# automl/TransformersCanDoBayesianInference

Measured on NVIDIA H100. Metric: prior-sampled sequences/sec, full training step (prior sample + fwd + bwd + allreduce + clip + Adam), higher is better.
Workload: dtype bf16

## Files before the change

transformerscandobayesianinference_b200/csrc/attention_bwd_tc.cu:

```cuda
#include "attention_common.cuh"

namespace pfn {

constexpr int AB_ROWS = ATT_TILE_ROWS;
constexpr int AB_TILE = ATT_TILE;
constexpr int AB_THREADS = 3 * 128;
constexpr int AB_DQ_STAGES = 4;
constexpr int AB_DKV_STAGES = 3;
constexpr int AB_DQ_STAT_WARPS = 3;
constexpr int AB_DQ_OFF_RING = 4 * AB_TILE;
constexpr int AB_DQ_OFF_STAT = AB_DQ_OFF_RING + AB_DQ_STAGES * 2 * AB_TILE;
constexpr int AB_DQ_OFF_BAR = AB_DQ_OFF_STAT + 2 * 3 * 128 * 4;
constexpr int AB_DQ_SMEM = AB_DQ_OFF_BAR + (2 * AB_DQ_STAGES + 2 + 4) * 8 + 1024;
constexpr int AB_DKV_OFF_RING = 4 * AB_TILE;
constexpr int AB_DKV_OFF_STAT = AB_DKV_OFF_RING + AB_DKV_STAGES * 2 * AB_TILE;
constexpr int AB_DKV_OFF_BAR = AB_DKV_OFF_STAT + AB_DKV_STAGES * 2 * AB_ROWS * 4;
constexpr int AB_DKV_SMEM = AB_DKV_OFF_BAR + (2 * AB_DKV_STAGES + 1) * 8 + 1024;
static_assert(AB_DQ_SMEM <= 232448 && AB_DKV_SMEM <= 232448, "the tiles and rings must fit the 227 KB of shared memory");

struct AttnBwdParams {
  int T, B, H, sep;
  float scale, scale_log2;
  const __nv_bfloat16* qkv; int ld_qkv;
  const __nv_bfloat16* dout; int ld_dout;
  __nv_bfloat16* dqkv; int ld_dqkv;
  const float* lse;
  const float* delta;
  int delta_tm;
  float* dq_colsum;
  uint32_t drop_seed; int drop_thr;
  int n_tiles;
  int batch_major;
};

__device__ __forceinline__ float ab_delta(const AttnBwdParams& p, int b, int h, int i) {
  return p.delta_tm ? p.delta[att_tok(i, b, p.T, p.B, 0) * p.H + h] : p.delta[(static_cast<size_t>(b) * p.H + h) * p.T + i];
}

__global__ void __launch_bounds__(256)
attn_bwd_delta_kernel(const __nv_bfloat16* __restrict__ out, int ld_out, const __nv_bfloat16* __restrict__ dout,
                      int ld_dout, float* __restrict__ delta, int T, int B, int H, int batch_major) {
  const int lane = threadIdx.x & 31;
  const long long warp = (static_cast<long long>(blockIdx.x) * blockDim.x + threadIdx.x) >> 5;
  const long long nwarps = (static_cast<long long>(gridDim.x) * blockDim.x) >> 5;
  const long long rows = static_cast<long long>(T) * B;
  for (long long tok = warp; tok < rows; tok += nwarps) {
    const int t = batch_major ? static_cast<int>(tok % T) : static_cast<int>(tok / B);
    const int b = batch_major ? static_cast<int>(tok / T) : static_cast<int>(tok % B);
    for (int h0 = 0; h0 < H; h0 += 2) {
      const int h = h0 + (lane >> 4);
      float acc = 0.f;
      if (h < H) {
        const int col = h * ATT_DH + (lane & 15) * 8;
        const uint4 pa = *reinterpret_cast<const uint4*>(out + tok * ld_out + col);
        const uint4 pb = *reinterpret_cast<const uint4*>(dout + tok * ld_dout + col);
        const __nv_bfloat162* ha = reinterpret_cast<const __nv_bfloat162*>(&pa);
        const __nv_bfloat162* hb = reinterpret_cast<const __nv_bfloat162*>(&pb);
#pragma unroll
        for (int j = 0; j < 4; ++j) {
          const float2 x = __bfloat1622float2(ha[j]);
          const float2 y = __bfloat1622float2(hb[j]);
          acc = fmaf(x.x, y.x, acc);
          acc = fmaf(x.y, y.y, acc);
        }
      }
#pragma unroll
      for (int o = 8; o > 0; o >>= 1) acc += __shfl_xor_sync(0xffffffffu, acc, o);
      if ((lane & 15) == 0 && h < H) delta[(static_cast<size_t>(b) * H + h) * T + t] = acc;
    }
  }
}

__global__ void __launch_bounds__(AB_THREADS, 1)
attn_bwd_dq_kernel(const __grid_constant__ CUtensorMap tmQ, const __grid_constant__ CUtensorMap tmKV,
                   const __grid_constant__ CUtensorMap tmDO, const AttnBwdParams p) {
  extern __shared__ uint8_t smem_raw[];
  uint8_t* smem = att_smem_base(smem_raw);
  uint8_t* sQ = smem;
  uint8_t* sD = smem + 2 * AB_TILE;
  const AttPipe<AB_DQ_STAGES> pp(smem + AB_DQ_OFF_RING, reinterpret_cast<uint64_t*>(smem + AB_DQ_OFF_BAR));
  float* sStat = reinterpret_cast<float*>(smem + AB_DQ_OFF_STAT);
  uint64_t* st_full = pp.q_empty + 1;
  uint64_t* st_empty = st_full + 2;
  const int warp = threadIdx.x >> 5, lane = threadIdx.x & 31;
  const int E = p.H * ATT_DH;
  const int nblk = (p.sep + AB_ROWS - 1) / AB_ROWS;
  const int n_units = p.n_tiles * p.B * p.H;
  const float dscale = p.drop_thr > 0 ? drop_scale(p.drop_thr) : 1.0f;
  if (threadIdx.x == 0) {
    pp.init();
    for (int s = 0; s < 2; ++s) {
      tc::mbar_init(&st_full[s], 32 * AB_DQ_STAT_WARPS);
      tc::mbar_init(&st_empty[s], 256);
    }
    tc::mbar_fence_init();
  }
  __syncthreads();

  if (warp >= 8) {
    tc::setmaxnreg_dec<64>();
    if (warp > 8) {
      const int pw = warp - 9;
      for (int u = blockIdx.x, it = 0; u < n_units; u += gridDim.x, ++it) {
        const AttUnit unit = att_unit(u, p.n_tiles, p.H);
        const int sb = it & 1;
        float* st = sStat + sb * 3 * 128;
        tc::mbar_wait_suspend(&st_empty[sb], ((it >> 1) & 1) ^ 1);
#pragma unroll 1
        for (int r = pw + AB_DQ_STAT_WARPS * lane; r < 128; r += 32 * AB_DQ_STAT_WARPS) {
          const int i = unit.tile * 128 + r;
          const bool valid = i < p.T;
          st[r] = valid ? p.lse[static_cast<size_t>(unit.bh) * p.T + i] * 1.4426950408889634f : INFINITY;
          st[128 + r] = valid ? ab_delta(p, unit.b, unit.h, i) : 0.f;
        }
        __syncwarp();
        auto tok_of = [&](int r) { return att_tok(unit.tile * 128 + r, unit.b, p.T, p.B, p.batch_major); };
        auto load_row = [&](int r, uint4& xv, uint4& yv) {
          const int l = static_cast<int>(att_opaque(lane)), half = l >> 4, c8 = (l & 15) * 8;
          const size_t tok = tok_of(r);
          const __nv_bfloat16* qrow = p.qkv + tok * p.ld_qkv + unit.h * ATT_DH + c8;
          xv = *reinterpret_cast<const uint4*>(half ? p.dout + tok * p.ld_dout + unit.h * ATT_DH + c8 : qrow);
          yv = *reinterpret_cast<const uint4*>(qrow + (1 + half) * E);
        };
        auto finish_row = [&](int r, uint4 xv, uint4 yv) {
          const int l = static_cast<int>(att_opaque(lane)), half = l >> 4, c8 = (l & 15) * 8;
          const __nv_bfloat162* x2 = reinterpret_cast<const __nv_bfloat162*>(&xv);
          const __nv_bfloat162* y2 = reinterpret_cast<const __nv_bfloat162*>(&yv);
          float dot = 0.f;
#pragma unroll
          for (int c = 0; c < 4; ++c) {
            const float2 a = __bfloat1622float2(x2[c]), bb = __bfloat1622float2(y2[c]);
            dot = fmaf(a.x, bb.x, fmaf(a.y, bb.y, dot));
          }
#pragma unroll
          for (int o = 8; o > 0; o >>= 1) dot += __shfl_xor_sync(0xffffffffu, dot, o);
          const float sd = __shfl_sync(0xffffffffu, dot, 0), dpd = __shfl_sync(0xffffffffu, dot, 16);
          const int i = unit.tile * 128 + r;
          const float pr = fast_ex2(fmaf(sd, p.scale_log2, -st[r]));
          const float mk = p.drop_thr > 0 ? (drop_keep(p.drop_seed, static_cast<uint32_t>(unit.bh) * p.T + i, i, p.drop_thr) ? dscale : 0.f) : 1.f;
          const float ds = pr * fmaf(mk, dpd, -st[128 + r]) * p.scale;
          const float f = half ? pr * mk : ds;
          uint4 o;
          uint32_t* o32 = reinterpret_cast<uint32_t*>(&o);
#pragma unroll
          for (int c = 0; c < 4; ++c) {
            const float2 a = __bfloat1622float2(x2[c]);
            o32[c] = tc::pack_bf16x2(f * a.x, f * a.y);
          }
          *reinterpret_cast<uint4*>(p.dqkv + tok_of(r) * p.ld_dqkv + unit.h * ATT_DH + (1 + half) * E + c8) = o;
          if (lane == 0) st[256 + r] = ds;
        };
        const int r_lo = max(0, p.sep - unit.tile * 128), r_hi = min(128, p.T - unit.tile * 128);
        for (int r = r_lo + (pw - r_lo % AB_DQ_STAT_WARPS + AB_DQ_STAT_WARPS) % AB_DQ_STAT_WARPS; r < r_hi;
             r += 2 * AB_DQ_STAT_WARPS) {
          const int r2 = r + AB_DQ_STAT_WARPS < r_hi ? r + AB_DQ_STAT_WARPS : r;
          uint4 xa, ya, xb, yb;
          load_row(r, xa, ya);
          load_row(r2, xb, yb);
          finish_row(r, xa, ya);
          if (r2 != r) finish_row(r2, xb, yb);
        }
        tc::mbar_arrive(&st_full[sb]);
      }
    } else if (threadIdx.x == 256) {
      tc::tma_prefetch_desc(&tmQ);
      tc::tma_prefetch_desc(&tmKV);
      tc::tma_prefetch_desc(&tmDO);
      att_kv_producer(pp, &tmKV, n_units, p.n_tiles, p.H, nblk, 4 * AB_TILE, [&](const AttUnit& unit) {
        for (int g = 0; g < 2; ++g) {
          const int t0 = unit.tile * 128 + 64 * g;
          att_load_tile(sQ + g * AB_TILE, &tmQ, pp.q_full, unit.h * ATT_DH, unit.b, t0);
          att_load_tile(sD + g * AB_TILE, &tmDO, pp.q_full, unit.h * ATT_DH, unit.b, t0);
        }
      });
    }
    return;
  }

  tc::setmaxnreg_inc<208>();
  const int g = warp >> 2, wq = warp & 3;
  const uint32_t q_tile = tc::smem_u32(sQ + g * AB_TILE), d_tile = tc::smem_u32(sD + g * AB_TILE);
  AttRing<AB_DQ_STAGES> ring;
  bool timed_out = false;
  for (int u = blockIdx.x, it = 0; u < n_units && !timed_out; u += gridDim.x, ++it) {
    const AttUnit unit = att_unit(u, p.n_tiles, p.H);
    const int i0 = unit.tile * 128 + 64 * g + 16 * wq + (lane >> 2);

    const int sb = it & 1;
    if (!tc::mbar_wait_bounded(&st_full[sb], (it >> 1) & 1)) { timed_out = true; break; }
    float lse2[2], dl[2], dsd[2];
    uint32_t drow[2];
#pragma unroll
    for (int r = 0; r < 2; ++r) {
      const int rr = i0 + 8 * r - unit.tile * 128;
      lse2[r] = sStat[sb * 3 * 128 + rr];
      dl[r] = sStat[sb * 3 * 128 + 128 + rr];
      dsd[r] = sStat[sb * 3 * 128 + 256 + rr];
      drow[r] = static_cast<uint32_t>(unit.bh) * p.T + i0 + 8 * r;
    }
    tc::mbar_arrive(&st_empty[sb]);

    float dq[64], s[32], dp[32];
    uint32_t ads[16];
    auto issue_sdp = [&](int st) {
      const uint32_t k_s = tc::smem_u32(pp.ring + st * 2 * AB_TILE);
      const uint32_t v_s = k_s + AB_TILE;
      const uint32_t q_s = att_opaque(q_tile), d_s = att_opaque(d_tile);
      tc::wgmma_fence();
#pragma unroll
      for (int kk = 0; kk < 8; ++kk) att_mma_n64(s, att_desc_k(q_s, kk), att_desc_k(k_s, kk), kk);
#pragma unroll
      for (int kk = 0; kk < 8; ++kk) att_mma_n64(dp, att_desc_k(d_s, kk), att_desc_k(v_s, kk), kk);
      tc::wgmma_commit();
    };
    auto issue_dq = [&](int st, bool accumulate) {
      const uint32_t k_s = tc::smem_u32(pp.ring + st * 2 * AB_TILE);
      tc::wgmma_fence();
#pragma unroll
      for (int kk = 0; kk < 4; ++kk) tc::wgmma_m64n128k16_rs(dq, ads + 4 * kk, att_desc_mn(k_s, kk), accumulate || kk > 0);
      tc::wgmma_commit();
    };
    auto compute_ds = [&](int kb) {
      const int key0 = kb * AB_ROWS + 2 * (lane & 3);
#pragma unroll
      for (int e = 0; e < 32; ++e) {
        const int r = (e >> 1) & 1;
        const int key = key0 + 8 * (e >> 2) + (e & 1);
        const float pr = key < p.sep ? fast_ex2(fmaf(s[e], p.scale_log2, -lse2[r])) : 0.f;
        const float mk = p.drop_thr > 0 ? (drop_keep(p.drop_seed, drow[r], key, p.drop_thr) ? dscale : 0.f) : 1.f;
        s[e] = pr * fmaf(mk, dp[e], -dl[r]) * p.scale;
      }
    };
    auto pack_ds = [&]() {
#pragma unroll
      for (int e = 0; e < 16; ++e) ads[e] = tc::pack_bf16x2(s[2 * e], s[2 * e + 1]);
    };
    uint32_t kd[2][16];
    auto load_kd = [&]() {
#pragma unroll
      for (int r = 0; r < 2; ++r) {
        const int i = i0 + 8 * r;
        const bool diag = i < p.T && i >= p.sep;
        const __nv_bfloat16* krow = p.qkv + att_tok(diag ? i : 0, unit.b, p.T, p.B, p.batch_major) * p.ld_qkv + E + unit.h * ATT_DH;
#pragma unroll
        for (int j = 0; j < 16; ++j)
          kd[r][j] = diag ? *reinterpret_cast<const uint32_t*>(krow + 8 * j + 2 * (lane & 3)) : 0u;
      }
    };
    if (att_key_loop(pp, ring, it, nblk, issue_sdp, issue_dq, [&] { tc::wgmma_fence_regs(s); tc::wgmma_fence_regs(dp); },
                     [&] { tc::wgmma_fence_regs(dq); }, compute_ds, pack_ds, load_kd)) {
      timed_out = true;
      break;
    }

    float cs[16][2];
#pragma unroll
    for (int j = 0; j < 16; ++j) cs[j][0] = cs[j][1] = 0.f;
#pragma unroll
    for (int r = 0; r < 2; ++r) {
      const int i = i0 + 8 * r;
      if (i < p.T) {
        const bool diag = i >= p.sep;
        __nv_bfloat16* grow = p.dqkv + att_tok(i, unit.b, p.T, p.B, p.batch_major) * p.ld_dqkv + unit.h * ATT_DH;
#pragma unroll
        for (int j = 0; j < 16; ++j) {
          float x = nblk > 0 ? dq[4 * j + 2 * r] : 0.f, y = nblk > 0 ? dq[4 * j + 2 * r + 1] : 0.f;
          if (diag) {
            const float2 k = __bfloat1622float2(*reinterpret_cast<const __nv_bfloat162*>(&kd[r][j]));
            x = fmaf(dsd[r], k.x, x);
            y = fmaf(dsd[r], k.y, y);
          }
          att_st2(grow, j, lane, x, y);
          cs[j][0] += __bfloat162float(__float2bfloat16_rn(x));
          cs[j][1] += __bfloat162float(__float2bfloat16_rn(y));
        }
      }
    }
    if (p.dq_colsum != nullptr) {
#pragma unroll
      for (int j = 0; j < 16; ++j)
#pragma unroll
        for (int e = 0; e < 2; ++e) {
          float v = cs[j][e];
          v += __shfl_xor_sync(0xffffffffu, v, 4);
          v += __shfl_xor_sync(0xffffffffu, v, 8);
          v += __shfl_xor_sync(0xffffffffu, v, 16);
          if (lane < 4) atomicAdd(p.dq_colsum + unit.h * ATT_DH + 8 * j + 2 * lane + e, v);
        }
    }
  }
  if (timed_out) asm volatile("trap;");
}

__global__ void __launch_bounds__(AB_THREADS, 1)
attn_bwd_dkv_kernel(const __grid_constant__ CUtensorMap tmQ, const __grid_constant__ CUtensorMap tmKV,
                    const __grid_constant__ CUtensorMap tmDO, const AttnBwdParams p) {
  extern __shared__ uint8_t smem_raw[];
  uint8_t* smem = att_smem_base(smem_raw);
  uint8_t* sK = smem;
  uint8_t* sV = smem + 2 * AB_TILE;
  uint8_t* sRing = smem + AB_DKV_OFF_RING;
  float* sStat = reinterpret_cast<float*>(smem + AB_DKV_OFF_STAT);
  uint64_t* full = reinterpret_cast<uint64_t*>(smem + AB_DKV_OFF_BAR);
  uint64_t* empty = full + AB_DKV_STAGES;
  uint64_t* kv_bar = empty + AB_DKV_STAGES;
  const int warp = threadIdx.x >> 5, lane = threadIdx.x & 31;
  const AttUnit unit = att_unit(blockIdx.x, p.n_tiles, p.H);
  const int E = p.H * ATT_DH;
  const int nqb = (p.T + AB_ROWS - 1) / AB_ROWS;
  if (threadIdx.x == 0) {
    for (int s = 0; s < AB_DKV_STAGES; ++s) {
      tc::mbar_init(&full[s], 1 + AB_ROWS);
      tc::mbar_init(&empty[s], 2);
    }
    tc::mbar_init(kv_bar, 1);
    tc::mbar_fence_init();
  }
  __syncthreads();

  if (warp >= 8) {
    tc::setmaxnreg_dec<40>();
    const int pt = threadIdx.x - 256;
    AttRing<AB_DKV_STAGES> ring;
    if (pt == 0) {
      tc::tma_prefetch_desc(&tmQ);
      tc::tma_prefetch_desc(&tmKV);
      tc::tma_prefetch_desc(&tmDO);
      tc::mbar_expect_tx(kv_bar, 4 * AB_TILE);
      for (int g = 0; g < 2; ++g) {
        const int j0 = unit.tile * 128 + 64 * g;
        att_load_tile(sK + g * AB_TILE, &tmKV, kv_bar, E + unit.h * ATT_DH, unit.b, j0);
        att_load_tile(sV + g * AB_TILE, &tmKV, kv_bar, 2 * E + unit.h * ATT_DH, unit.b, j0);
// ... 149 lines not shown
```

transformerscandobayesianinference_b200/csrc/attention_common.cuh:

```cuda
#pragma once
#include "common.cuh"
#include "dropout.cuh"
#include "tc_common.cuh"
#include "../../include/pfn_b200.h"

namespace pfn {

constexpr int ATT_DH = 128;
constexpr int ATT_ROW_BYTES = ATT_DH * 2;
constexpr int ATT_TILE_ROWS = 64;
constexpr int ATT_TILE = ATT_TILE_ROWS * ATT_ROW_BYTES;

int check_attn_desc_public(const pfn_attn_desc* d, bool bwd, const char* who);

__device__ __forceinline__ size_t att_tok(int t, int b, int T, int B, int batch_major) {
  return batch_major ? static_cast<size_t>(b) * T + t : static_cast<size_t>(t) * B + b;
}

__device__ __forceinline__ uint64_t att_desc_k(uint32_t tile, int kk) {
  return tc::wgmma_smem_desc(tile + (kk >> 2) * 8192 + (kk & 3) * 32, 16, 1024);
}
__device__ __forceinline__ uint64_t att_desc_mn(uint32_t tile, int kk) {
  return tc::wgmma_smem_desc(tile + kk * 2048, 8192, 1024);
}
__device__ __forceinline__ uint32_t att_opaque(uint32_t addr) {
  asm volatile("" : "+r"(addr));
  return addr;
}
__device__ __forceinline__ void att_mma_n64(float (&d)[32], uint64_t a_desc, uint64_t b_desc, int kk) {
  if (kk == 0) tc::wgmma_m64n64k16<0>(d, a_desc, b_desc);
  else tc::wgmma_m64n64k16<1>(d, a_desc, b_desc);
}

__device__ __forceinline__ void att_load_tile(uint8_t* dst, const CUtensorMap* m, uint64_t* bar, int col0, int b, int t0) {
  tc::tma_load_3d(dst, m, bar, col0, b, t0);
  tc::tma_load_3d(dst + 8192, m, bar, col0 + 64, b, t0);
}

struct AttUnit {
  int tile;
  int bh, h, b;
};
__device__ __forceinline__ AttUnit att_unit(int u, int n_tiles, int H) {
  const int bh = u / n_tiles;
  return {u % n_tiles, bh, bh % H, bh / H};
}

template <int STAGES>
struct AttRing {
  int stage = 0;
  uint32_t phase = 0;
  __device__ __forceinline__ void advance() { if (++stage == STAGES) { stage = 0; phase ^= 1; } }
};

__device__ __forceinline__ uint8_t* att_smem_base(uint8_t* raw) {
  return raw + ((1024u - (tc::smem_u32(raw) & 1023u)) & 1023u);
}

template <int STAGES>
struct AttPipe {
  uint8_t* ring;
  uint64_t* kv_full;
  uint64_t* kv_empty;
  uint64_t* q_full;
  uint64_t* q_empty;
  __device__ __forceinline__ AttPipe(uint8_t* ring_smem, uint64_t* bars)
      : ring(ring_smem), kv_full(bars), kv_empty(bars + STAGES), q_full(bars + 2 * STAGES), q_empty(bars + 2 * STAGES + 1) {}
  __device__ __forceinline__ void init() const {
    for (int s = 0; s < STAGES; ++s) {
      tc::mbar_init(&kv_full[s], 1);
      tc::mbar_init(&kv_empty[s], 2);
    }
    tc::mbar_init(q_full, 1);
    tc::mbar_init(q_empty, 2);
  }
};

template <int STAGES, class LoadQ>
__device__ __forceinline__ void att_kv_producer(const AttPipe<STAGES>& pp, const CUtensorMap* tmKV, int n_units, int n_tiles,
                                                int H, int nblk, uint32_t q_bytes, LoadQ&& load_q) {
  const int E = H * ATT_DH;
  AttRing<STAGES> ring;
  for (int u = blockIdx.x, it = 0; u < n_units; u += gridDim.x, ++it) {
    const AttUnit unit = att_unit(u, n_tiles, H);
    auto claim_q = [&]() {
      if (it > 0) tc::mbar_wait_suspend(pp.q_empty, (it - 1) & 1);
      tc::mbar_expect_tx(pp.q_full, q_bytes);
      load_q(unit);
    };
    const int claim_at = min(STAGES - 1, nblk - 1);
    if (nblk == 0) claim_q();
    for (int kb = 0; kb < nblk; ++kb) {
      if (kb == claim_at) claim_q();
      tc::mbar_wait_suspend(&pp.kv_empty[ring.stage], ring.phase ^ 1);
      uint8_t* dst = pp.ring + ring.stage * 2 * ATT_TILE;
      tc::mbar_expect_tx(&pp.kv_full[ring.stage], 2 * ATT_TILE);
      att_load_tile(dst, tmKV, &pp.kv_full[ring.stage], E + unit.h * ATT_DH, unit.b, kb * ATT_TILE_ROWS);
      att_load_tile(dst + ATT_TILE, tmKV, &pp.kv_full[ring.stage], 2 * E + unit.h * ATT_DH, unit.b, kb * ATT_TILE_ROWS);
      ring.advance();
    }
  }
}

template <int STAGES, class IssueA, class IssueB, class FenceA, class FenceB, class Math, class Pack, class BeforeTail>
__device__ __forceinline__ bool att_key_loop(const AttPipe<STAGES>& pp, AttRing<STAGES>& ring, int it, int nblk,
                                             IssueA&& issue_a, IssueB&& issue_b, FenceA&& fence_a, FenceB&& fence_b,
                                             Math&& math, Pack&& pack, BeforeTail&& before_tail) {
  const bool leader = (threadIdx.x & 127) == 0;
  if (!tc::mbar_wait_bounded(pp.q_full, it & 1)) return true;
  if (nblk > 0) {
    if (!tc::mbar_wait_bounded(&pp.kv_full[ring.stage], ring.phase)) return true;
    issue_a(ring.stage);
    tc::wgmma_wait<0>();
    fence_a();
    if (nblk == 1 && leader) tc::mbar_arrive(pp.q_empty);
    math(0);
    pack();
    int cur = ring.stage;
    ring.advance();
    bool timed_out = false;
    for (int kb = 1; kb < nblk; ++kb) {
      if (!timed_out && !tc::mbar_wait_bounded(&pp.kv_full[ring.stage], ring.phase)) timed_out = true;
      issue_a(ring.stage);
      issue_b(cur, kb > 1);
      tc::wgmma_wait<1>();
      fence_a();
      if (kb == nblk - 1 && leader) tc::mbar_arrive(pp.q_empty);
      math(kb);
      tc::wgmma_wait<0>();
      fence_b();
      if (leader) tc::mbar_arrive(&pp.kv_empty[cur]);
      cur = ring.stage;
      ring.advance();
      pack();
    }
    issue_b(cur, nblk > 1);
    before_tail();
    tc::wgmma_wait<0>();
    fence_b();
    if (timed_out) return true;
    if (leader) tc::mbar_arrive(&pp.kv_empty[cur]);
  } else {
    if (leader) tc::mbar_arrive(pp.q_empty);
    before_tail();
  }
  return false;
}

__device__ __forceinline__ float2 att_ld2(const __nv_bfloat16* row, int j, int lane) {
  return __bfloat1622float2(*reinterpret_cast<const __nv_bfloat162*>(row + 8 * j + 2 * (lane & 3)));
}
__device__ __forceinline__ void att_st2(__nv_bfloat16* row, int j, int lane, float x, float y) {
  *reinterpret_cast<uint32_t*>(row + 8 * j + 2 * (lane & 3)) = tc::pack_bf16x2(x, y);
}
__device__ __forceinline__ float quad_sum(float v) {
  v += __shfl_xor_sync(0xffffffffu, v, 1);
  return v + __shfl_xor_sync(0xffffffffu, v, 2);
}
__device__ __forceinline__ float quad_max(float v) {
  v = fmaxf(v, __shfl_xor_sync(0xffffffffu, v, 1));
  return fmaxf(v, __shfl_xor_sync(0xffffffffu, v, 2));
}

static inline int check_tc_attn(const pfn_attn_desc* d, bool bwd, const char* who) {
  if (int rc = check_attn_desc_public(d, bwd, who)) return rc;
  PFN_CHECK_ARG(d->dtype == PFN_BF16, "%s: bf16 only", who);
  PFN_CHECK_ARG(d->dh == ATT_DH, "%s: head dim %d unsupported (built for 128)", who, d->dh);
  PFN_CHECK_ARG(d->ld_qkv % 8 == 0 && d->ld_out % 8 == 0, "%s: leading dims must be multiples of 8", who);
  PFN_CHECK_ARG(((reinterpret_cast<uintptr_t>(d->qkv) | reinterpret_cast<uintptr_t>(d->out)) & 15) == 0,
                "%s: qkv/out must be 16-byte aligned", who);
  if (bwd) {
    PFN_CHECK_ARG(d->ld_dout % 8 == 0 && d->ld_dqkv % 8 == 0, "%s: leading dims must be multiples of 8", who);
    PFN_CHECK_ARG(((reinterpret_cast<uintptr_t>(d->dout) | reinterpret_cast<uintptr_t>(d->dqkv)) & 15) == 0,
                  "%s: dout/dqkv must be 16-byte aligned", who);
  }
  return 0;
}

template <auto Kernel, class... Args>
static inline int att_launch_persistent(const char* who, long long units, int threads, int smem, cudaStream_t s,
                                        const Args&... args) {
  PFN_CHECK_ARG(units < (1LL << 31), "%s: too many tiles", who);
  static bool attr_set[64] = {};
  if (first_use_on_device(attr_set)) PFN_CUDA_OK(cudaFuncSetAttribute(Kernel, cudaFuncAttributeMaxDynamicSharedMemorySize, smem));
  const int grid = units < num_sms() ? static_cast<int>(units) : num_sms();
  Kernel<<<static_cast<unsigned>(grid), threads, smem, s>>>(args...);
  PFN_LAUNCH_OK();
  return 0;
}

static inline int att_tensor_map(CUtensorMap* m, const void* base, int cols, int ld, int T, int B, int t_extent,
                                 int batch_major) {
  const uint64_t row = static_cast<uint64_t>(ld) * 2;
  const uint64_t dims[3] = {static_cast<uint64_t>(cols), static_cast<uint64_t>(B), static_cast<uint64_t>(t_extent)};
  const uint64_t strides[3] = {0, batch_major ? row * T : row, batch_major ? row : row * B};
  const uint32_t box[3] = {64, 1, ATT_TILE_ROWS};
  return make_tensor_map(m, base, false, 3, dims, strides, box, true);
}

static inline int att_qkv_maps(const pfn_attn_desc* d, CUtensorMap* tmQ, CUtensorMap* tmKV) {
  const int E = d->H * ATT_DH;
  if (int rc = att_tensor_map(tmQ, d->qkv, 3 * E, d->ld_qkv, d->T, d->B, d->T, d->batch_major)) return rc;
  return att_tensor_map(tmKV, d->qkv, 3 * E, d->ld_qkv, d->T, d->B, d->sep > 0 ? d->sep : 1, d->batch_major);
}

}
```

transformerscandobayesianinference_b200/csrc/attention_tc.cu:

```cuda
#include "attention_common.cuh"

namespace pfn {

constexpr int AF_THREADS = 3 * 128;
constexpr int AF_STAGES = 4;
constexpr int AF_OFF_STG = 2 * ATT_TILE;
constexpr int AF_OFF_RING = 4 * ATT_TILE;
constexpr int AF_OFF_BAR = AF_OFF_RING + AF_STAGES * 2 * ATT_TILE;
constexpr int AF_SMEM = AF_OFF_BAR + (2 * AF_STAGES + 2) * 8 + 1024;
static_assert(AF_SMEM <= 232448, "the tiles and the ring must fit the 227 KB of shared memory");

struct AttnFwdParams {
  int T, B, H, sep;
  float scale_log2;
  const __nv_bfloat16* qkv; int ld_qkv;
  float* lse;
  int n_tiles;
  int batch_major;
  uint32_t drop_seed; int drop_thr;
};

__global__ void __launch_bounds__(AF_THREADS, 1)
attn_fwd_kernel(const __grid_constant__ CUtensorMap tmQ, const __grid_constant__ CUtensorMap tmKV,
                const __grid_constant__ CUtensorMap tmO, const AttnFwdParams p) {
  extern __shared__ uint8_t smem_raw[];
  uint8_t* smem = att_smem_base(smem_raw);
  uint8_t* sQ = smem;
  uint8_t* sStg = smem + AF_OFF_STG;
  const AttPipe<AF_STAGES> pp(smem + AF_OFF_RING, reinterpret_cast<uint64_t*>(smem + AF_OFF_BAR));
  const int warp = threadIdx.x >> 5, lane = threadIdx.x & 31;
  const int E = p.H * ATT_DH;
  const int nblk = (p.sep + ATT_TILE_ROWS - 1) / ATT_TILE_ROWS;
  const int n_units = p.n_tiles * p.B * p.H;
  if (threadIdx.x == 0) {
    pp.init();
    tc::mbar_fence_init();
  }
  __syncthreads();

  if (warp >= 8) {
    tc::setmaxnreg_dec<40>();
    if (threadIdx.x == 256) {
      tc::tma_prefetch_desc(&tmQ);
      tc::tma_prefetch_desc(&tmKV);
      att_kv_producer(pp, &tmKV, n_units, p.n_tiles, p.H, nblk, 2 * ATT_TILE, [&](const AttUnit& unit) {
        for (int g = 0; g < 2; ++g)
          att_load_tile(sQ + g * ATT_TILE, &tmQ, pp.q_full, unit.h * ATT_DH, unit.b, unit.tile * 128 + 64 * g);
      });
    }
    return;
  }

  tc::setmaxnreg_inc<232>();
  const int g = warp >> 2, wq = warp & 3;
  const int tid = threadIdx.x & 127;
  const uint32_t q_tile = tc::smem_u32(sQ + g * ATT_TILE);
  uint8_t* stg = sStg + g * ATT_TILE;
  const float dscale = p.drop_thr > 0 ? drop_scale(p.drop_thr) : 1.0f;
  AttRing<AF_STAGES> ring;
  bool timed_out = false;
  for (int u = blockIdx.x, it = 0; u < n_units && !timed_out; u += gridDim.x, ++it) {
    const AttUnit unit = att_unit(u, p.n_tiles, p.H);
    const int t0 = unit.tile * 128 + 64 * g;
    const int i0 = t0 + 16 * wq + (lane >> 2);

    float o[64], m[2], l[2];
    uint32_t drow[2];
#pragma unroll
    for (int r = 0; r < 2; ++r) {
      const int i = i0 + 8 * r;
      const bool diag = i < p.T && i >= p.sep;
      drow[r] = static_cast<uint32_t>(unit.bh) * p.T + i;
      const __nv_bfloat16* qrow = p.qkv + att_tok(diag ? i : 0, unit.b, p.T, p.B, p.batch_major) * p.ld_qkv + unit.h * ATT_DH;
      float sd = 0.f;
      if (diag) {
#pragma unroll
        for (int j = 0; j < 16; ++j) {
          const float2 q = att_ld2(qrow, j, lane), k = att_ld2(qrow + E, j, lane);
          sd = fmaf(q.x, k.x, fmaf(q.y, k.y, sd));
        }
      }
      sd = quad_sum(sd) * p.scale_log2;
      m[r] = diag ? sd : -INFINITY;
      l[r] = diag && (lane & 3) == 0 ? 1.f : 0.f;
      const bool keep = diag && (p.drop_thr == 0 || drop_keep(p.drop_seed, drow[r], i, p.drop_thr));
#pragma unroll
      for (int j = 0; j < 16; ++j) {
        const float2 v = keep ? att_ld2(qrow + 2 * E, j, lane) : make_float2(0.f, 0.f);
        o[4 * j + 2 * r] = v.x;
        o[4 * j + 2 * r + 1] = v.y;
      }
    }

    float s[32];
    uint32_t ap[16];
    float corr[2];
    auto issue_s = [&](int st) {
      const uint32_t k_s = tc::smem_u32(pp.ring + st * 2 * ATT_TILE);
      const uint32_t q_s = att_opaque(q_tile);
      tc::wgmma_fence();
#pragma unroll
      for (int kk = 0; kk < 8; ++kk) att_mma_n64(s, att_desc_k(q_s, kk), att_desc_k(k_s, kk), kk);
      tc::wgmma_commit();
    };
    auto issue_pv = [&](int st, bool) {
      const uint32_t v_s = tc::smem_u32(pp.ring + st * 2 * ATT_TILE) + ATT_TILE;
      tc::wgmma_fence();
#pragma unroll
      for (int kk = 0; kk < 4; ++kk) tc::wgmma_m64n128k16_rs(o, ap + 4 * kk, att_desc_mn(v_s, kk), 1);
      tc::wgmma_commit();
    };
    auto softmax = [&](int kb) {
      const int key0 = kb * ATT_TILE_ROWS + 2 * (lane & 3);
      if (kb * ATT_TILE_ROWS + ATT_TILE_ROWS > p.sep) {
#pragma unroll
        for (int e = 0; e < 32; ++e)
          if (key0 + 8 * (e >> 2) + (e & 1) >= p.sep) s[e] = -INFINITY;
      }
      float mx[2] = {-INFINITY, -INFINITY};
#pragma unroll
      for (int e = 0; e < 32; ++e) mx[(e >> 1) & 1] = fmaxf(mx[(e >> 1) & 1], s[e]);
#pragma unroll
      for (int r = 0; r < 2; ++r) {
        const float mn = fmaxf(m[r], quad_max(mx[r]) * p.scale_log2);
        corr[r] = fast_ex2(m[r] - mn);
        m[r] = mn;
        l[r] *= corr[r];
      }
#pragma unroll
      for (int e = 0; e < 32; ++e) {
        const int r = (e >> 1) & 1;
        const float pr = fast_ex2(fmaf(s[e], p.scale_log2, -m[r]));
        l[r] += pr;
        s[e] = p.drop_thr > 0 && !drop_keep(p.drop_seed, drow[r], key0 + 8 * (e >> 2) + (e & 1), p.drop_thr) ? 0.f : pr;
      }
    };
    auto rescale_pack = [&]() {
#pragma unroll
      for (int e = 0; e < 64; ++e) o[e] *= corr[(e >> 1) & 1];
#pragma unroll
      for (int e = 0; e < 16; ++e) ap[e] = tc::pack_bf16x2(s[2 * e], s[2 * e + 1]);
    };
    if (att_key_loop(pp, ring, it, nblk, issue_s, issue_pv, [&] { tc::wgmma_fence_regs(s); },
                     [&] { tc::wgmma_fence_regs(o); }, softmax, rescale_pack, [] {})) {
      timed_out = true;
      break;
    }

    if (tid == 0) tc::bulk_wait_read<0>();
    tc::named_bar_sync(1 + g, 128);
#pragma unroll
    for (int r = 0; r < 2; ++r) {
      const int i = i0 + 8 * r;
      const float lr = quad_sum(l[r]);
      const float inv = dscale / lr;
      const int rr = 16 * wq + (lane >> 2) + 8 * r;
#pragma unroll
      for (int j = 0; j < 16; ++j) {
        const uint32_t off = (j >> 3) * 8192 + rr * 128 + (((j & 7) ^ (rr & 7)) << 4) + (lane & 3) * 4;
        *reinterpret_cast<uint32_t*>(stg + off) = tc::pack_bf16x2(o[4 * j + 2 * r] * inv, o[4 * j + 2 * r + 1] * inv);
      }
      if (i < p.T && (lane & 3) == 0) p.lse[static_cast<size_t>(unit.bh) * p.T + i] = (m[r] + __log2f(lr)) * 0.69314718055994531f;
    }
    tc::fence_proxy_async_smem();
    tc::named_bar_sync(1 + g, 128);
    if (tid == 0 && t0 < p.T) {
      tc::tma_store_3d(&tmO, stg, unit.h * ATT_DH, unit.b, t0);
      tc::tma_store_3d(&tmO, stg + 8192, unit.h * ATT_DH + 64, unit.b, t0);
      tc::bulk_commit();
    }
  }
  if (tid == 0) tc::bulk_wait<0>();
  if (timed_out) asm volatile("trap;");
}

}

using namespace pfn;

extern "C" int pfn_attention_fwd_tc(const pfn_attn_desc* d, void* stream) {
  if (int rc = check_tc_attn(d, false, "attention_fwd_tc")) return rc;
  AttnFwdParams p;
  p.T = d->T; p.B = d->B; p.H = d->H; p.sep = d->sep;
  p.scale_log2 = d->scale * 1.4426950408889634f;
  p.qkv = reinterpret_cast<const __nv_bfloat16*>(d->qkv); p.ld_qkv = d->ld_qkv;
  p.lse = d->lse;
  p.n_tiles = (d->T + 127) / 128;
  p.batch_major = d->batch_major;
  p.drop_seed = d->drop_seed; p.drop_thr = d->drop_thr;
  const int E = d->H * ATT_DH;
  CUtensorMap tmQ, tmKV, tmO;
  if (int rc = att_qkv_maps(d, &tmQ, &tmKV)) return rc;
  if (int rc = att_tensor_map(&tmO, d->out, E, d->ld_out, d->T, d->B, d->T, d->batch_major)) return rc;
  return att_launch_persistent<attn_fwd_kernel>("attention_fwd_tc", static_cast<long long>(p.n_tiles) * d->B * d->H,
                                                AF_THREADS, AF_SMEM, reinterpret_cast<cudaStream_t>(stream), tmQ, tmKV, tmO, p);
}
```

transformerscandobayesianinference_b200/csrc/tc_common.cuh:

```cuda
#pragma once
#include <cuda.h>
#include <cuda_bf16.h>
#include <cuda_runtime.h>
#include <stdint.h>

namespace pfn {
namespace tc {

__device__ __forceinline__ uint32_t smem_u32(const void* p) {
  return static_cast<uint32_t>(__cvta_generic_to_shared(p));
}

__device__ __forceinline__ void mbar_init(uint64_t* bar, uint32_t count) {
  asm volatile("mbarrier.init.shared::cta.b64 [%0], %1;" ::"r"(smem_u32(bar)), "r"(count) : "memory");
}
__device__ __forceinline__ void mbar_fence_init() {
  asm volatile("fence.mbarrier_init.release.cluster;" ::: "memory");
}
__device__ __forceinline__ void mbar_expect_tx(uint64_t* bar, uint32_t bytes) {
  asm volatile("mbarrier.arrive.expect_tx.shared::cta.b64 _, [%0], %1;" ::"r"(smem_u32(bar)), "r"(bytes) : "memory");
}
__device__ __forceinline__ void mbar_arrive(uint64_t* bar) {
  asm volatile("mbarrier.arrive.shared::cta.b64 _, [%0];" ::"r"(smem_u32(bar)) : "memory");
}
// ... 71 lines not shown
}
__device__ __forceinline__ void bulk_commit() { asm volatile("cp.async.bulk.commit_group;" ::: "memory"); }
template <int N>
__device__ __forceinline__ void bulk_wait_read() {
  asm volatile("cp.async.bulk.wait_group.read %0;" ::"n"(N) : "memory");
}
template <int N>
__device__ __forceinline__ void bulk_wait() {
  asm volatile("cp.async.bulk.wait_group %0;" ::"n"(N) : "memory");
}
__device__ __forceinline__ void fence_proxy_async_smem() { asm volatile("fence.proxy.async.shared::cta;" ::: "memory"); }

__device__ __forceinline__ void named_bar_sync(int id, int threads) {
  asm volatile("bar.sync %0, %1;" ::"r"(id), "r"(threads) : "memory");
}
__device__ __forceinline__ void named_bar_arrive(int id, int threads) {
  asm volatile("bar.arrive %0, %1;" ::"r"(id), "r"(threads) : "memory");
}
template <int N>
__device__ __forceinline__ void setmaxnreg_dec() { asm volatile("setmaxnreg.dec.sync.aligned.u32 %0;" ::"n"(N)); }
template <int N>
__device__ __forceinline__ void setmaxnreg_inc() { asm volatile("setmaxnreg.inc.sync.aligned.u32 %0;" ::"n"(N)); }

__device__ __forceinline__ uint32_t pack_bf16x2(float lo, float hi) {
  __nv_bfloat162 t = __floats2bfloat162_rn(lo, hi);
  return *reinterpret_cast<uint32_t*>(&t);
}

__device__ __forceinline__ uint64_t wgmma_smem_desc(uint32_t smem_addr, uint32_t lbo_bytes, uint32_t sbo_bytes) {
  return (1ull << 62) | (static_cast<uint64_t>((sbo_bytes >> 4) & 0x3FFF) << 32) |
         (static_cast<uint64_t>((lbo_bytes >> 4) & 0x3FFF) << 16) | static_cast<uint64_t>((smem_addr >> 4) & 0x3FFF);
}

__device__ __forceinline__ void wgmma_fence() { asm volatile("wgmma.fence.sync.aligned;" ::: "memory"); }
__device__ __forceinline__ void wgmma_commit() { asm volatile("wgmma.commit_group.sync.aligned;" ::: "memory"); }
template <int N>
__device__ __forceinline__ void wgmma_wait() {
  asm volatile("wgmma.wait_group.sync.aligned %0;" ::"n"(N) : "memory");
}
template <int N>
__device__ __forceinline__ void wgmma_fence_regs(float (&d)[N]) {
#pragma unroll
  for (int i = 0; i < N; ++i) asm volatile("" : "+f"(d[i])::"memory");
}

template <int TA, int TB>
__device__ __forceinline__ void wgmma_m64n128k16(float (&d)[64], uint64_t a_desc, uint64_t b_desc, uint32_t accumulate) {
  asm volatile(
      "{\n\t.reg .pred p;\n\t"
      "setp.ne.b32 p, %66, 0;\n\t"
      "wgmma.mma_async.sync.aligned.m64n128k16.f32.bf16.bf16 "
      "{%0, %1, %2, %3, %4, %5, %6, %7, %8, %9, %10, %11, %12, %13, %14, %15, "
      "%16, %17, %18, %19, %20, %21, %22, %23, %24, %25, %26, %27, %28, %29, %30, %31, "
      "%32, %33, %34, %35, %36, %37, %38, %39, %40, %41, %42, %43, %44, %45, %46, %47, "
      "%48, %49, %50, %51, %52, %53, %54, %55, %56, %57, %58, %59, %60, %61, %62, %63}, "
      "%64, %65, p, 1, 1, %67, %68;\n\t}"
      : "+f"(d[0]), "+f"(d[1]), "+f"(d[2]), "+f"(d[3]), "+f"(d[4]), "+f"(d[5]), "+f"(d[6]), "+f"(d[7]),
        "+f"(d[8]), "+f"(d[9]), "+f"(d[10]), "+f"(d[11]), "+f"(d[12]), "+f"(d[13]), "+f"(d[14]), "+f"(d[15]),
        "+f"(d[16]), "+f"(d[17]), "+f"(d[18]), "+f"(d[19]), "+f"(d[20]), "+f"(d[21]), "+f"(d[22]), "+f"(d[23]),
        "+f"(d[24]), "+f"(d[25]), "+f"(d[26]), "+f"(d[27]), "+f"(d[28]), "+f"(d[29]), "+f"(d[30]), "+f"(d[31]),
        "+f"(d[32]), "+f"(d[33]), "+f"(d[34]), "+f"(d[35]), "+f"(d[36]), "+f"(d[37]), "+f"(d[38]), "+f"(d[39]),
        "+f"(d[40]), "+f"(d[41]), "+f"(d[42]), "+f"(d[43]), "+f"(d[44]), "+f"(d[45]), "+f"(d[46]), "+f"(d[47]),
        "+f"(d[48]), "+f"(d[49]), "+f"(d[50]), "+f"(d[51]), "+f"(d[52]), "+f"(d[53]), "+f"(d[54]), "+f"(d[55]),
        "+f"(d[56]), "+f"(d[57]), "+f"(d[58]), "+f"(d[59]), "+f"(d[60]), "+f"(d[61]), "+f"(d[62]), "+f"(d[63])
      : "l"(a_desc), "l"(b_desc), "r"(accumulate), "n"(TA), "n"(TB));
}

#define PFN_WGMMA_D32(C)                                                                                          \
  C(d[0]), C(d[1]), C(d[2]), C(d[3]), C(d[4]), C(d[5]), C(d[6]), C(d[7]), C(d[8]), C(d[9]), C(d[10]), C(d[11]),   \
      C(d[12]), C(d[13]), C(d[14]), C(d[15]), C(d[16]), C(d[17]), C(d[18]), C(d[19]), C(d[20]), C(d[21]),         \
      C(d[22]), C(d[23]), C(d[24]), C(d[25]), C(d[26]), C(d[27]), C(d[28]), C(d[29]), C(d[30]), C(d[31])
#define PFN_WGMMA_M64N64K16(SCALE_D)                                                                              \
  "wgmma.mma_async.sync.aligned.m64n64k16.f32.bf16.bf16 "                                                         \
  "{%0, %1, %2, %3, %4, %5, %6, %7, %8, %9, %10, %11, %12, %13, %14, %15, "                                       \
  "%16, %17, %18, %19, %20, %21, %22, %23, %24, %25, %26, %27, %28, %29, %30, %31}, %32, %33, " SCALE_D ", 1, 1, 0, 0;"
template <int ACCUMULATE>
__device__ __forceinline__ void wgmma_m64n64k16(float (&d)[32], uint64_t a_desc, uint64_t b_desc) {
  if constexpr (ACCUMULATE) {
    asm volatile(PFN_WGMMA_M64N64K16("1") : PFN_WGMMA_D32("+f") : "l"(a_desc), "l"(b_desc));
  } else {
    asm volatile(PFN_WGMMA_M64N64K16("0") : PFN_WGMMA_D32("=f") : "l"(a_desc), "l"(b_desc));
  }
}
#undef PFN_WGMMA_M64N64K16
#undef PFN_WGMMA_D32

__device__ __forceinline__ void wgmma_m64n128k16_rs(float (&d)[64], const uint32_t* a, uint64_t b_desc, uint32_t accumulate) {
  asm volatile(
      "{\n\t.reg .pred p;\n\t"
      "setp.ne.b32 p, %69, 0;\n\t"
      "wgmma.mma_async.sync.aligned.m64n128k16.f32.bf16.bf16 "
      "{%0, %1, %2, %3, %4, %5, %6, %7, %8, %9, %10, %11, %12, %13, %14, %15, "
      "%16, %17, %18, %19, %20, %21, %22, %23, %24, %25, %26, %27, %28, %29, %30, %31, "
      "%32, %33, %34, %35, %36, %37, %38, %39, %40, %41, %42, %43, %44, %45, %46, %47, "
      "%48, %49, %50, %51, %52, %53, %54, %55, %56, %57, %58, %59, %60, %61, %62, %63}, "
      "{%64, %65, %66, %67}, %68, p, 1, 1, 1;\n\t}"
      : "+f"(d[0]), "+f"(d[1]), "+f"(d[2]), "+f"(d[3]), "+f"(d[4]), "+f"(d[5]), "+f"(d[6]), "+f"(d[7]),
        "+f"(d[8]), "+f"(d[9]), "+f"(d[10]), "+f"(d[11]), "+f"(d[12]), "+f"(d[13]), "+f"(d[14]), "+f"(d[15]),
        "+f"(d[16]), "+f"(d[17]), "+f"(d[18]), "+f"(d[19]), "+f"(d[20]), "+f"(d[21]), "+f"(d[22]), "+f"(d[23]),
        "+f"(d[24]), "+f"(d[25]), "+f"(d[26]), "+f"(d[27]), "+f"(d[28]), "+f"(d[29]), "+f"(d[30]), "+f"(d[31]),
        "+f"(d[32]), "+f"(d[33]), "+f"(d[34]), "+f"(d[35]), "+f"(d[36]), "+f"(d[37]), "+f"(d[38]), "+f"(d[39]),
        "+f"(d[40]), "+f"(d[41]), "+f"(d[42]), "+f"(d[43]), "+f"(d[44]), "+f"(d[45]), "+f"(d[46]), "+f"(d[47]),
        "+f"(d[48]), "+f"(d[49]), "+f"(d[50]), "+f"(d[51]), "+f"(d[52]), "+f"(d[53]), "+f"(d[54]), "+f"(d[55]),
        "+f"(d[56]), "+f"(d[57]), "+f"(d[58]), "+f"(d[59]), "+f"(d[60]), "+f"(d[61]), "+f"(d[62]), "+f"(d[63])
      : "r"(a[0]), "r"(a[1]), "r"(a[2]), "r"(a[3]), "l"(b_desc), "r"(accumulate));
}

}

int make_tensor_map(CUtensorMap* out, const void* base, bool f32, int rank, const uint64_t* dims,
                    const uint64_t* strides_bytes, const uint32_t* box, bool swizzle128);

}
```

Baseline: 3354.

## Hold Q in registers for QK^T wgmma and release Q buffer early

The attention forward and backward-dQ kernels now load the Q tile into registers with ldmatrix once per unit and issue QK^T as register-sourced wgmma, so the Q shared-memory buffer can be released right after the first key block. The forward kernel then lets the producer prefetch the next Q tile sooner, and its diagonal (self-token) term is loaded during the key loop and folded in as an online-softmax update after the loop rather than before it. The dQ kernel raises its register budget to hold the extra 32 Q registers but keeps the late Q release. This adds register pressure and a possible risk of spills.

```diff
diff --git a/transformerscandobayesianinference_b200/csrc/attention_bwd_tc.cu b/transformerscandobayesianinference_b200/csrc/attention_bwd_tc.cu
--- a/transformerscandobayesianinference_b200/csrc/attention_bwd_tc.cu
+++ b/transformerscandobayesianinference_b200/csrc/attention_bwd_tc.cu
@@ -78,7 +78,7 @@
   uint8_t* smem = att_smem_base(smem_raw);
   uint8_t* sQ = smem;
   uint8_t* sD = smem + 2 * AB_TILE;
-  const AttPipe<AB_DQ_STAGES> pp(smem + AB_DQ_OFF_RING, reinterpret_cast<uint64_t*>(smem + AB_DQ_OFF_BAR));
+  const AttPipe<AB_DQ_STAGES, false> pp(smem + AB_DQ_OFF_RING, reinterpret_cast<uint64_t*>(smem + AB_DQ_OFF_BAR));
   float* sStat = reinterpret_cast<float*>(smem + AB_DQ_OFF_STAT);
   uint64_t* st_full = pp.q_empty + 1;
   uint64_t* st_empty = st_full + 2;
@@ -177,7 +177,7 @@
     return;
   }
 
-  tc::setmaxnreg_inc<208>();
+  tc::setmaxnreg_inc<216>();
   const int g = warp >> 2, wq = warp & 3;
   const uint32_t q_tile = tc::smem_u32(sQ + g * AB_TILE), d_tile = tc::smem_u32(sD + g * AB_TILE);
   AttRing<AB_DQ_STAGES> ring;
@@ -201,14 +201,15 @@
     tc::mbar_arrive(&st_empty[sb]);
 
     float dq[64], s[32], dp[32];
-    uint32_t ads[16];
+    uint32_t qa[32], ads[16];
+    auto load_q = [&] { att_load_a(qa, q_tile, wq, lane); };
     auto issue_sdp = [&](int st) {
       const uint32_t k_s = tc::smem_u32(pp.ring + st * 2 * AB_TILE);
       const uint32_t v_s = k_s + AB_TILE;
-      const uint32_t q_s = att_opaque(q_tile), d_s = att_opaque(d_tile);
+      const uint32_t d_s = att_opaque(d_tile);
       tc::wgmma_fence();
 #pragma unroll
-      for (int kk = 0; kk < 8; ++kk) att_mma_n64(s, att_desc_k(q_s, kk), att_desc_k(k_s, kk), kk);
+      for (int kk = 0; kk < 8; ++kk) att_mma_n64_rs(s, qa, att_desc_k(k_s, kk), kk);
 #pragma unroll
       for (int kk = 0; kk < 8; ++kk) att_mma_n64(dp, att_desc_k(d_s, kk), att_desc_k(v_s, kk), kk);
       tc::wgmma_commit();
@@ -247,7 +248,7 @@
           kd[r][j] = diag ? *reinterpret_cast<const uint32_t*>(krow + 8 * j + 2 * (lane & 3)) : 0u;
       }
     };
-    if (att_key_loop(pp, ring, it, nblk, issue_sdp, issue_dq, [&] { tc::wgmma_fence_regs(s); tc::wgmma_fence_regs(dp); },
+    if (att_key_loop(pp, ring, it, nblk, load_q, issue_sdp, issue_dq, [&] { tc::wgmma_fence_regs(s); tc::wgmma_fence_regs(dp); },
                      [&] { tc::wgmma_fence_regs(dq); }, compute_ds, pack_ds, load_kd)) {
       timed_out = true;
       break;
diff --git a/transformerscandobayesianinference_b200/csrc/attention_common.cuh b/transformerscandobayesianinference_b200/csrc/attention_common.cuh
--- a/transformerscandobayesianinference_b200/csrc/attention_common.cuh
+++ b/transformerscandobayesianinference_b200/csrc/attention_common.cuh
@@ -30,6 +30,18 @@
 __device__ __forceinline__ void att_mma_n64(float (&d)[32], uint64_t a_desc, uint64_t b_desc, int kk) {
   if (kk == 0) tc::wgmma_m64n64k16<0>(d, a_desc, b_desc);
   else tc::wgmma_m64n64k16<1>(d, a_desc, b_desc);
+}
+__device__ __forceinline__ void att_mma_n64_rs(float (&d)[32], const uint32_t (&a)[32], uint64_t b_desc, int kk) {
+  if (kk == 0) tc::wgmma_m64n64k16_rs<0>(d, a + 4 * kk, b_desc);
+  else tc::wgmma_m64n64k16_rs<1>(d, a + 4 * kk, b_desc);
+}
+__device__ __forceinline__ void att_load_a(uint32_t (&a)[32], uint32_t tile, int wq, int lane) {
+  const uint32_t row = tile + (16 * wq + (lane & 7) + 8 * ((lane >> 3) & 1)) * 128;
+#pragma unroll
+  for (int kk = 0; kk < 8; ++kk) {
+    const int c = 2 * (kk & 3) + (lane >> 4);
+    tc::ldmatrix_x4(a + 4 * kk, row + (kk >> 2) * 8192 + ((c ^ (lane & 7)) << 4));
+  }
 }
 
 __device__ __forceinline__ void att_load_tile(uint8_t* dst, const CUtensorMap* m, uint64_t* bar, int col0, int b, int t0) {
@@ -57,7 +69,7 @@
   return raw + ((1024u - (tc::smem_u32(raw) & 1023u)) & 1023u);
 }
 
-template <int STAGES>
+template <int STAGES, bool Q_IN_REGS>
 struct AttPipe {
   uint8_t* ring;
   uint64_t* kv_full;
@@ -76,9 +88,9 @@
   }
 };
 
-template <int STAGES, class LoadQ>
-__device__ __forceinline__ void att_kv_producer(const AttPipe<STAGES>& pp, const CUtensorMap* tmKV, int n_units, int n_tiles,
-                                                int H, int nblk, uint32_t q_bytes, LoadQ&& load_q) {
+template <int STAGES, bool Q_IN_REGS, class LoadQ>
+__device__ __forceinline__ void att_kv_producer(const AttPipe<STAGES, Q_IN_REGS>& pp, const CUtensorMap* tmKV, int n_units,
+                                                int n_tiles, int H, int nblk, uint32_t q_bytes, LoadQ&& load_q) {
   const int E = H * ATT_DH;
   AttRing<STAGES> ring;
   for (int u = blockIdx.x, it = 0; u < n_units; u += gridDim.x, ++it) {
@@ -88,7 +100,7 @@
       tc::mbar_expect_tx(pp.q_full, q_bytes);
       load_q(unit);
     };
-    const int claim_at = min(STAGES - 1, nblk - 1);
+    const int claim_at = Q_IN_REGS ? 0 : min(STAGES - 1, nblk - 1);
     if (nblk == 0) claim_q();
     for (int kb = 0; kb < nblk; ++kb) {
       if (kb == claim_at) claim_q();
@@ -102,18 +114,20 @@
   }
 }
 
-template <int STAGES, class IssueA, class IssueB, class FenceA, class FenceB, class Math, class Pack, class BeforeTail>
-__device__ __forceinline__ bool att_key_loop(const AttPipe<STAGES>& pp, AttRing<STAGES>& ring, int it, int nblk,
-                                             IssueA&& issue_a, IssueB&& issue_b, FenceA&& fence_a, FenceB&& fence_b,
-                                             Math&& math, Pack&& pack, BeforeTail&& before_tail) {
+template <int STAGES, bool Q_IN_REGS, class LoadA, class IssueA, class IssueB, class FenceA, class FenceB, class Math,
+          class Pack, class BeforeTail>
+__device__ __forceinline__ bool att_key_loop(const AttPipe<STAGES, Q_IN_REGS>& pp, AttRing<STAGES>& ring, int it, int nblk,
+                                             LoadA&& load_a, IssueA&& issue_a, IssueB&& issue_b, FenceA&& fence_a,
+                                             FenceB&& fence_b, Math&& math, Pack&& pack, BeforeTail&& before_tail) {
   const bool leader = (threadIdx.x & 127) == 0;
   if (!tc::mbar_wait_bounded(pp.q_full, it & 1)) return true;
   if (nblk > 0) {
+    load_a();
     if (!tc::mbar_wait_bounded(&pp.kv_full[ring.stage], ring.phase)) return true;
     issue_a(ring.stage);
     tc::wgmma_wait<0>();
     fence_a();
-    if (nblk == 1 && leader) tc::mbar_arrive(pp.q_empty);
+    if ((Q_IN_REGS || nblk == 1) && leader) tc::mbar_arrive(pp.q_empty);
     math(0);
     pack();
     int cur = ring.stage;
@@ -125,7 +139,7 @@
       issue_b(cur, kb > 1);
       tc::wgmma_wait<1>();
       fence_a();
-      if (kb == nblk - 1 && leader) tc::mbar_arrive(pp.q_empty);
+      if (!Q_IN_REGS && kb == nblk - 1 && leader) tc::mbar_arrive(pp.q_empty);
       math(kb);
       tc::wgmma_wait<0>();
       fence_b();
diff --git a/transformerscandobayesianinference_b200/csrc/attention_tc.cu b/transformerscandobayesianinference_b200/csrc/attention_tc.cu
--- a/transformerscandobayesianinference_b200/csrc/attention_tc.cu
+++ b/transformerscandobayesianinference_b200/csrc/attention_tc.cu
@@ -27,7 +27,7 @@
   uint8_t* smem = att_smem_base(smem_raw);
   uint8_t* sQ = smem;
   uint8_t* sStg = smem + AF_OFF_STG;
-  const AttPipe<AF_STAGES> pp(smem + AF_OFF_RING, reinterpret_cast<uint64_t*>(smem + AF_OFF_BAR));
+  const AttPipe<AF_STAGES, true> pp(smem + AF_OFF_RING, reinterpret_cast<uint64_t*>(smem + AF_OFF_BAR));
   const int warp = threadIdx.x >> 5, lane = threadIdx.x & 31;
   const int E = p.H * ATT_DH;
   const int nblk = (p.sep + ATT_TILE_ROWS - 1) / ATT_TILE_ROWS;
@@ -68,39 +68,22 @@
     uint32_t drow[2];
 #pragma unroll
     for (int r = 0; r < 2; ++r) {
-      const int i = i0 + 8 * r;
-      const bool diag = i < p.T && i >= p.sep;
-      drow[r] = static_cast<uint32_t>(unit.bh) * p.T + i;
-      const __nv_bfloat16* qrow = p.qkv + att_tok(diag ? i : 0, unit.b, p.T, p.B, p.batch_major) * p.ld_qkv + unit.h * ATT_DH;
-      float sd = 0.f;
-      if (diag) {
-#pragma unroll
-        for (int j = 0; j < 16; ++j) {
-          const float2 q = att_ld2(qrow, j, lane), k = att_ld2(qrow + E, j, lane);
-          sd = fmaf(q.x, k.x, fmaf(q.y, k.y, sd));
-        }
-      }
-      sd = quad_sum(sd) * p.scale_log2;
-      m[r] = diag ? sd : -INFINITY;
-      l[r] = diag && (lane & 3) == 0 ? 1.f : 0.f;
-      const bool keep = diag && (p.drop_thr == 0 || drop_keep(p.drop_seed, drow[r], i, p.drop_thr));
-#pragma unroll
-      for (int j = 0; j < 16; ++j) {
-        const float2 v = keep ? att_ld2(qrow + 2 * E, j, lane) : make_float2(0.f, 0.f);
-        o[4 * j + 2 * r] = v.x;
-        o[4 * j + 2 * r + 1] = v.y;
-      }
-    }
+      drow[r] = static_cast<uint32_t>(unit.bh) * p.T + i0 + 8 * r;
+      m[r] = -INFINITY;
+      l[r] = 0.f;
+    }
+#pragma unroll
+    for (int e = 0; e < 64; ++e) o[e] = 0.f;
 
     float s[32];
-    uint32_t ap[16];
+    uint32_t qa[32], ap[16];
     float corr[2];
+    auto load_q = [&] { att_load_a(qa, q_tile, wq, lane); };
     auto issue_s = [&](int st) {
       const uint32_t k_s = tc::smem_u32(pp.ring + st * 2 * ATT_TILE);
-      const uint32_t q_s = att_opaque(q_tile);
       tc::wgmma_fence();
 #pragma unroll
-      for (int kk = 0; kk < 8; ++kk) att_mma_n64(s, att_desc_k(q_s, kk), att_desc_k(k_s, kk), kk);
+      for (int kk = 0; kk < 8; ++kk) att_mma_n64_rs(s, qa, att_desc_k(k_s, kk), kk);
       tc::wgmma_commit();
     };
     auto issue_pv = [&](int st, bool) {
@@ -141,26 +124,67 @@
 #pragma unroll
       for (int e = 0; e < 16; ++e) ap[e] = tc::pack_bf16x2(s[2 * e], s[2 * e + 1]);
     };
-    if (att_key_loop(pp, ring, it, nblk, issue_s, issue_pv, [&] { tc::wgmma_fence_regs(s); },
-                     [&] { tc::wgmma_fence_regs(o); }, softmax, rescale_pack, [] {})) {
+    uint32_t qd[2][16], kd[2][16], vd[2][16];
+    auto load_diag = [&]() {
+#pragma unroll
+      for (int r = 0; r < 2; ++r) {
+        const int i = i0 + 8 * r;
+        const bool diag = i < p.T && i >= p.sep;
+        const bool keep = diag && (p.drop_thr == 0 || drop_keep(p.drop_seed, drow[r], i, p.drop_thr));
+        const __nv_bfloat16* qrow = p.qkv + att_tok(diag ? i : 0, unit.b, p.T, p.B, p.batch_major) * p.ld_qkv +
+                                    unit.h * ATT_DH + 2 * (lane & 3);
+#pragma unroll
+        for (int j = 0; j < 16; ++j) {
+          qd[r][j] = diag ? *reinterpret_cast<const uint32_t*>(qrow + 8 * j) : 0u;
+          kd[r][j] = diag ? *reinterpret_cast<const uint32_t*>(qrow + E + 8 * j) : 0u;
+          vd[r][j] = keep ? *reinterpret_cast<const uint32_t*>(qrow + 2 * E + 8 * j) : 0u;
+        }
+      }
+    };
+    if (att_key_loop(pp, ring, it, nblk, load_q, issue_s, issue_pv, [&] { tc::wgmma_fence_regs(s); },
+                     [&] { tc::wgmma_fence_regs(o); }, softmax, rescale_pack, load_diag)) {
       timed_out = true;
       break;
     }
 
+    float lr[2];
+#pragma unroll
+    for (int r = 0; r < 2; ++r) {
+      const int i = i0 + 8 * r;
+      float sd = 0.f;
+#pragma unroll
+      for (int j = 0; j < 16; ++j) {
+        const float2 q = __bfloat1622float2(*reinterpret_cast<const __nv_bfloat162*>(&qd[r][j]));
+        const float2 k = __bfloat1622float2(*reinterpret_cast<const __nv_bfloat162*>(&kd[r][j]));
+        sd = fmaf(q.x, k.x, fmaf(q.y, k.y, sd));
+      }
+      sd = quad_sum(sd) * p.scale_log2;
+      if (i >= p.T || i < p.sep) sd = -INFINITY;
+      const float mn = fmaxf(m[r], sd);
+      const float c = fast_ex2(m[r] - mn), pd = fast_ex2(sd - mn);
+      lr[r] = fmaf(quad_sum(l[r]), c, pd);
+      m[r] = mn;
+#pragma unroll
+      for (int j = 0; j < 16; ++j) {
+        const float2 v = __bfloat1622float2(*reinterpret_cast<const __nv_bfloat162*>(&vd[r][j]));
+        o[4 * j + 2 * r] = fmaf(o[4 * j + 2 * r], c, pd * v.x);
+        o[4 * j + 2 * r + 1] = fmaf(o[4 * j + 2 * r + 1], c, pd * v.y);
+      }
+    }
+
     if (tid == 0) tc::bulk_wait_read<0>();
     tc::named_bar_sync(1 + g, 128);
 #pragma unroll
     for (int r = 0; r < 2; ++r) {
       const int i = i0 + 8 * r;
-      const float lr = quad_sum(l[r]);
-      const float inv = dscale / lr;
+      const float inv = dscale / lr[r];
       const int rr = 16 * wq + (lane >> 2) + 8 * r;
 #pragma unroll
       for (int j = 0; j < 16; ++j) {
         const uint32_t off = (j >> 3) * 8192 + rr * 128 + (((j & 7) ^ (rr & 7)) << 4) + (lane & 3) * 4;
         *reinterpret_cast<uint32_t*>(stg + off) = tc::pack_bf16x2(o[4 * j + 2 * r] * inv, o[4 * j + 2 * r + 1] * inv);
       }
-      if (i < p.T && (lane & 3) == 0) p.lse[static_cast<size_t>(unit.bh) * p.T + i] = (m[r] + __log2f(lr)) * 0.69314718055994531f;
+      if (i < p.T && (lane & 3) == 0) p.lse[static_cast<size_t>(unit.bh) * p.T + i] = (m[r] + __log2f(lr[r])) * 0.69314718055994531f;
     }
     tc::fence_proxy_async_smem();
     tc::named_bar_sync(1 + g, 128);
diff --git a/transformerscandobayesianinference_b200/csrc/tc_common.cuh b/transformerscandobayesianinference_b200/csrc/tc_common.cuh
--- a/transformerscandobayesianinference_b200/csrc/tc_common.cuh
+++ b/transformerscandobayesianinference_b200/csrc/tc_common.cuh
@@ -177,8 +177,31 @@
     asm volatile(PFN_WGMMA_M64N64K16("0") : PFN_WGMMA_D32("=f") : "l"(a_desc), "l"(b_desc));
   }
 }
+#define PFN_WGMMA_M64N64K16_RS(SCALE_D)                                                                           \
+  "wgmma.mma_async.sync.aligned.m64n64k16.f32.bf16.bf16 "                                                         \
+  "{%0, %1, %2, %3, %4, %5, %6, %7, %8, %9, %10, %11, %12, %13, %14, %15, "                                       \
+  "%16, %17, %18, %19, %20, %21, %22, %23, %24, %25, %26, %27, %28, %29, %30, %31}, "                             \
+  "{%32, %33, %34, %35}, %36, " SCALE_D ", 1, 1, 0;"
+template <int ACCUMULATE>
+__device__ __forceinline__ void wgmma_m64n64k16_rs(float (&d)[32], const uint32_t* a, uint64_t b_desc) {
+  if constexpr (ACCUMULATE) {
+    asm volatile(PFN_WGMMA_M64N64K16_RS("1") : PFN_WGMMA_D32("+f")
+                 : "r"(a[0]), "r"(a[1]), "r"(a[2]), "r"(a[3]), "l"(b_desc));
+  } else {
+    asm volatile(PFN_WGMMA_M64N64K16_RS("0") : PFN_WGMMA_D32("=f")
+                 : "r"(a[0]), "r"(a[1]), "r"(a[2]), "r"(a[3]), "l"(b_desc));
+  }
+}
+#undef PFN_WGMMA_M64N64K16_RS
 #undef PFN_WGMMA_M64N64K16
 #undef PFN_WGMMA_D32
+
+__device__ __forceinline__ void ldmatrix_x4(uint32_t* r, uint32_t addr) {
+  asm volatile("ldmatrix.sync.aligned.m8n8.x4.shared.b16 {%0, %1, %2, %3}, [%4];"
+               : "=r"(r[0]), "=r"(r[1]), "=r"(r[2]), "=r"(r[3])
+               : "r"(addr)
+               : "memory");
+}
 
 __device__ __forceinline__ void wgmma_m64n128k16_rs(float (&d)[64], const uint32_t* a, uint64_t b_desc, uint32_t accumulate) {
   asm volatile(
```

Measured after the change: 3363, median of 6. About the same (+0.2%).
